# shangfuu/avse_challenge

Measured on AMD Instinct MI355X. Metric: utterances/sec (3s@16kHz + 75 lip frames), higher is better.
Workload: dtype fp32; 1 GPU; avse1 AV baseline train step (BASELINE configs[1]): HIP STFT front-end + AVNet (ResNet18 lip enc + TCN, dilated Conv2d audio net, LSTM fusion) fwd/bwd + Adam; global_batch=32, per_gpu_batch=32, seq_len=48000, stft_frames=376, lip_frames=75, lip_hw=96, parallelism=dp1, hip_graph=fwd+bwd+opt

## Files before the change

### avse_challenge_amd/_lib.py

```python
import ctypes
import os

import torch

_HERE = os.path.dirname(os.path.abspath(__file__))
LIB_PATH = os.environ.get("AVSE_HIP_LIB", os.path.join(_HERE, "libavse_hip.so"))

c_i64, c_i32, c_f32, c_vp = ctypes.c_int64, ctypes.c_int32, ctypes.c_float, ctypes.c_void_p

AVSE_F32, AVSE_BF16 = 0, 1


class ScanFwdArgs(ctypes.Structure):
    _fields_ = [
        ("batch", c_i64), ("dim", c_i64), ("seqlen", c_i64), ("dstate", c_i64),
        ("in_dtype", c_i32), ("delta_softplus", c_i32), ("reverse", c_i32),
        ("u", c_vp), ("u_bs", c_i64), ("u_ds", c_i64),
        ("delta", c_vp), ("delta_bs", c_i64), ("delta_ds", c_i64),
        ("A", c_vp),
        ("B", c_vp), ("B_bs", c_i64), ("B_ns", c_i64),
        ("C", c_vp), ("C_bs", c_i64), ("C_ns", c_i64),
        ("D", c_vp),
        ("z", c_vp), ("z_bs", c_i64), ("z_ds", c_i64),
        ("delta_bias", c_vp),
# ... 167 lines not shown
    "avse_dwconv_gln_fwd": (c_i32, [c_i64] * 5 + [c_vp] * 5 + [c_f32] + [c_vp] * 5),
    "avse_dwconv_gln_fwd_q": (c_i32, [c_i64] * 5 + [c_vp] * 5 + [c_f32] + [c_vp] * 3 + [c_i64] + [c_vp] * 4),
    "avse_dwconv_gln_bwd": (c_i32, [c_i64] * 5 + [c_vp] * 14),
    "avse_prelu_gln_fwd_len": (c_i32, [c_i64] * 3 + [c_vp] * 5 + [c_f32] + [c_vp] * 4),
    "avse_dwconv_gln_fwd_len": (c_i32, [c_i64] * 5 + [c_vp] * 6 + [c_f32] + [c_vp] * 5),
    "avse_dwconv_gln_fwd_q_len": (c_i32, [c_i64] * 5 + [c_vp] * 6 + [c_f32] + [c_vp] * 3 + [c_i64] + [c_vp] * 4),
    "avse_dwconv_fwd_len": (c_i32, [c_i64] * 5 + [c_vp] * 5),
    "avse_upsample_linear_len": (c_i32, [c_i64] * 5 + [c_vp, c_i64, c_i64, c_vp, c_vp, c_vp, c_i64, c_i64, c_vp]),
    "avse_lstm_padded_hidden": (c_i64, [c_i64]),
    "avse_lstm_group_size": (c_i64, [c_i64, c_i64]),
    "avse_lstm_group_workspace_bytes": (c_i64, [c_i64, c_i64]),
    "avse_lstm_group_capacity": (c_i64, [c_i64, c_i32]),
    "avse_lstm_fwd_group": (c_i32, [c_i64, c_i64, c_i64, c_i32, c_vp, c_vp, c_vp, c_i64, c_i64, c_vp, c_vp, c_vp, c_vp,
                                    c_vp]),
    "avse_lstm_bwd_group": (c_i32, [c_i64, c_i64, c_i64, c_i32, c_vp, c_i64, c_i64, c_vp, c_vp, c_vp, c_vp, c_vp, c_vp,
                                    c_vp]),
    "avse_lstm_fwd": (c_i32, [c_i64, c_i64, c_i64, c_i32, c_vp, c_vp, c_vp, c_i64, c_i64, c_vp, c_vp, c_vp]),
    "avse_lstm_bwd": (c_i32, [c_i64, c_i64, c_i64, c_i32, c_vp, c_i64, c_i64, c_vp, c_vp, c_vp, c_vp, c_vp]),
    "avse_gemm_bf16": (c_i32, [ctypes.POINTER(GemmBf16Args), c_vp]),
    "avse_gemm_f32s": (c_i32, [ctypes.POINTER(GemmF32sArgs), c_vp]),
    "avse_split16_planes": (c_i32, [c_i64, c_i64, c_i64, c_vp, c_i64, c_i64, c_vp, c_vp, c_vp, c_vp]),
    "avse_add_max": (c_i32, [c_i64, c_i64, c_i64, c_vp, c_vp, c_vp, c_vp, c_vp]),
    "avse_split16_planes_known": (c_i32, [c_i64, c_i64, c_i64, c_vp, c_i64, c_i64, c_vp, c_vp, c_vp, c_vp]),
    "avse_split16_planes_to": (c_i32, [c_i64, c_i64, c_i64, c_vp, c_i64, c_i64, c_vp, c_vp, c_i64, c_i64, c_vp, c_i32,
                                       c_vp]),
    "avse_dconv_wprep_bytes": (c_i64, []),
    "avse_split16": (c_i32, [c_i64, c_vp, c_vp, c_vp, c_vp]),
    "avse_split16_known": (c_i32, [c_i64, c_vp, c_vp, c_vp, c_vp]),
    "avse_dconv_wprep": (c_i32, [c_vp, c_i32, c_vp, c_vp, c_vp]),
    "avse_dconv_fwd": (c_i32, [c_i64, c_i64, c_i64, c_i64, c_vp, c_vp, c_vp, c_vp, c_vp, c_vp]),
    "avse_dconv_wprep2": (c_i32, [c_vp] * 6),
    "avse_dconv_wgrad16_workspace_bytes": (c_i64, [c_i64, c_i64, c_i64]),
    "avse_dconv_wgrad16": (c_i32, [c_i64, c_i64, c_i64, c_i64, c_vp, c_vp, c_vp, c_vp, c_vp, c_vp, c_vp, c_vp]),
    "avse_conv1_fwd": (c_i32, [c_i64] * 3 + [c_vp] * 5),
    "avse_conv1_dgrad": (c_i32, [c_i64] * 3 + [c_vp] * 4),
    "avse_conv1_wgrad_workspace_bytes": (c_i64, [c_i64] * 3),
    "avse_conv1_wgrad": (c_i32, [c_i64] * 3 + [c_vp] * 6),
    "avse_convf_fwd": (c_i32, [c_i64] + [c_vp] * 5),
    "avse_convf_dgrad": (c_i32, [c_i64] + [c_vp] * 4),
    "avse_convf_wgrad_workspace_bytes": (c_i64, [c_i64]),
    "avse_convf_wgrad": (c_i32, [c_i64] + [c_vp] * 6),
    "avse_sconv_wprep_bytes": (c_i64, [c_i64, c_i64]),
    "avse_sconv_wprep": (c_i32, [c_i64, c_i64, c_vp, c_i32, c_vp, c_vp, c_vp]),
    "avse_sconv_fwd": (c_i32, [c_i64] * 6 + [c_vp] * 6),
    "avse_sconv_wgrad_workspace_bytes": (c_i64, [c_i64] * 6),
    "avse_sconv_wgrad": (c_i32, [c_i64] * 6 + [c_vp] * 7),
    "avse_sconv_dgrad2_supported": (c_i32, [c_i64] * 5),
    "avse_sconv_dgrad2": (c_i32, [c_i64] * 5 + [c_vp] * 6),
    "avse_mbstoi_frames": (c_i64, [c_i64]),
    "avse_mbstoi_workspace_bytes": (c_i64, [c_i64, c_i64]),
    "avse_mbstoi_gate": (c_i32, [c_i64, c_i64] + [c_vp] * 7),
    "avse_mbstoi_bands": (c_i32, [c_i64, c_i64] + [c_vp] * 6),
    "avse_mbstoi_ec": (c_i32, [c_i64, c_i64, c_vp, c_i32, c_i64, c_i64] + [c_vp] * 8),
    "avse_mbstoi_score": (c_i32, [c_i64, c_i64, c_vp, c_i32, c_vp, c_vp, c_vp]),
}

_lib = None


class HipLibraryError(RuntimeError):
    pass


ABI_VERSION = 2


# ... 34 lines not shown
```

### avse_challenge_amd/csrc/dconv.hip

```cpp
#include <algorithm>

#include "bnact_cols.h"
#include "common.h"
#include "split16.h"

namespace avse {
namespace dcf {

typedef _Float16 half8 __attribute__((ext_vector_type(8)));
typedef float floatx16 __attribute__((ext_vector_type(16)));

constexpr int C = 64, KS = 5, NQ = 4, TP = 256, THREADS = 256, WAVES = THREADS / 64;
constexpr int ROWB = 64;
constexpr int WIMG = KS * C * ROWB;
constexpr int NSTG = KS * NQ;
constexpr int MAXD = 16;
constexpr int XIMG_MAX = (TP + 8 * MAXD) * ROWB;
constexpr int STAGE = XIMG_MAX + WIMG;
constexpr int NBUF = 3;
constexpr int MAXP = (XIMG_MAX + WIMG) / 1024 / WAVES + 1;
static_assert(NBUF * STAGE <= 160 * 1024, "LDS");

__device__ inline int swz(int r) { return (r >> 2) & 3; }

// ... 158 lines not shown
    const float scale = __builtin_ldexpf(1.f, -(split_exp(a.maxbits[0]) + split_exp(a.maxbits[1])));
    auto store = [&](int j) {
        const int o = 32 * j + (lane & 31);
        const float bv = a.bias ? a.bias[o] : 0.f;
#pragma unroll
        for (int i = 0; i < 2; ++i)
#pragma unroll
            for (int g = 0; g < 4; ++g)
#pragma unroll
                for (int e = 0; e < 4; ++e) {
                    const int p = p0 + 64 * wave + 32 * i + 8 * g + 4 * (lane >> 5) + e;
                    const float v = acc[i][j][4 * g + e] * scale + bv;
                    if constexpr (EPI != 0) acc[i][j][4 * g + e] = v;
                    if (p < HW) a.y[((int64_t)n * HW + p) * C + o] = v;
                }
    };
    if constexpr (EPI == 0) {
#pragma unroll
        for (int j = 0; j < 2; ++j) store(j);
    } else {
        constexpr int ENQ = EPI == 2 ? 4 : 3;
        float* part = reinterpret_cast<float*>(lds);
        __syncthreads();
        bnact::bn_epi_wave<bnact::ACT_RELU, EPI == 2>(
            a.bn, [&](int i, int j, int r) { return acc[i][j][r]; }, store, (int64_t)n * HW + p0 + 64 * wave,
            (int64_t)(n + 1) * HW, 0, C, lane, part + wave * ENQ * 64);
        __syncthreads();
        bnact::bn_epi_row<EPI == 2>(a.bn, part, NW, 1, (int64_t)bid, 0, C);
    }
}

constexpr int WG_CHUNK = 64;
constexpr int PIXB = 256;
constexpr int WTHREADS = 512, WWAVES = WTHREADS / 64;

typedef short s4_t __attribute__((ext_vector_type(4)));
typedef __attribute__((address_space(3))) s4_t lds_s4_t;

__device__ inline int tswz(int r, int c) { return c ^ (((r & 1) << 1) | ((r & 2) << 2)); }

__device__ inline half8 tfrag(const uint8_t* img, const int (&row)[2], int cb, int pl, int lane) {
    const int g = lane >> 4, i = lane & 15;
    const int q = 2 * cb + (g & 1);
    s4_t v[2];
#pragma unroll
    for (int u = 0; u < 2; ++u) {
        const int r = row[u];
        const int byte = q * 64 + pl * 32 + 8 * (i & 3);
        const int off = r * PIXB + 16 * tswz(r, byte >> 4) + (byte & 15);
        v[u] = __builtin_amdgcn_ds_read_tr16_b64_v4i16((lds_s4_t*)(img + off));
    }
    const s4_t w0 = v[0], w1 = v[1];
    const short __attribute__((ext_vector_type(8))) w = {w0[0], w0[1], w0[2], w0[3], w1[0], w1[1], w1[2], w1[3]};
    return __builtin_bit_cast(half8, w);
}

struct WArgs {
    const void* xq;
    const void* dyq;
    const uint32_t* xmax;
    const uint32_t* dymax;
    float* part;
    float* dbpart;
    int N, H, W, cpi, chunks, ranges;
};

struct ChunkPos {
    int n, p0, hA, wA0;
    __device__ void init(int c, int cpi, int W) {
        n = c / cpi;
        p0 = (c - n * cpi) * WG_CHUNK;
        hA = p0 / W;
        wA0 = p0 - hA * W;
    }
    __device__ void next(int HW, int W) {
        p0 += WG_CHUNK;
        if (p0 >= HW) {
            ++n;
            p0 = hA = wA0 = 0;
        } else {
            wA0 += WG_CHUNK;
            if (wA0 >= W) {
                wA0 -= W;
                ++hA;
            }
        }
    }
};

template <int D>
__global__ __launch_bounds__(WTHREADS, 1) void wgrad_kernel(WArgs a) {
    constexpr int NP = WG_CHUNK + 8 * D;
    constexpr int YIMG = WG_CHUNK * PIXB, XIMG = NP * PIXB, STG = YIMG + XIMG;
    constexpr int NB = (3 * STG <= 160 * 1024) ? 3 : 2;
    constexpr int PY = YIMG / 1024, PT = PY + XIMG / 1024;
    constexpr int MAXPW = PT / WWAVES + 1;
    __shared__ __attribute__((aligned(1024))) uint8_t lds[NB * STG];
    const int lane = threadIdx.x & 63;
    const int wave = __builtin_amdgcn_readfirstlane(threadIdx.x >> 6);
    const int bid = xcd_remap(blockIdx.x, gridDim.x);
    const int r = bid / KS, kh = bid % KS;
    const int c_lo = (int)((int64_t)r * a.chunks / a.ranges), c_hi = (int)((int64_t)(r + 1) * a.chunks / a.ranges);
    const int HW = a.H * a.W;
    const i4_t rx = dma_rsrc(a.xq, (int64_t)a.N * HW * PIXB);
    const i4_t ry = dma_rsrc(a.dyq, (int64_t)a.N * HW * PIXB);
    const uint32_t lds0 = lds_u32(lds);
    const int npieces = (PT - wave + WWAVES - 1) / WWAVES;
    const int pr = lane >> 4, pc = lane & 15;
    int pj[MAXPW];
    uint32_t psw[MAXPW];
#pragma unroll
    for (int m = 0; m < MAXPW; ++m) {
        const int k = wave + WWAVES * m;
        pj[m] = k < PY ? 4 * k + pr : 4 * (k - PY) + pr;
        psw[m] = 16u * tswz(pj[m], pc);
    }

    auto issue = [&](const ChunkPos& cp, int buf) {
        const int nA = min(WG_CHUNK, a.W - cp.wA0);
        const int row1 = cp.hA + D * (kh - 2), row2 = nA < WG_CHUNK ? row1 + 1 : -1000000;
        const int ybase = cp.n * HW + cp.p0;
        const int nHrow = cp.n * a.H;
        const uint32_t img = lds0 + buf * STG;
#pragma unroll
        for (int m = 0; m < MAXPW; ++m) {
            if (m >= npieces) break;
            const int k = wave + WWAVES * m;
            if (k < PY) {
                const int j = pj[m];
                const uint32_t off = cp.p0 + j < HW ? (uint32_t)(ybase + j) * PIXB + psw[m] : 0x7FFFFFF0u;
                dma16(ry, img + k * 1024, off);
            } else {
                const int q = pj[m];
                const bool s1 = q < nA + 4 * D;
                const int col = s1 ? cp.wA0 - 2 * D + q : q - nA - 6 * D;
                const int row = s1 ? row1 : row2;
                const bool ok = (unsigned)col < (unsigned)a.W && (unsigned)row < (unsigned)a.H;
                const uint32_t pix = (uint32_t)((nHrow + row) * a.W + col);
                dma16(rx, img + YIMG + (k - PY) * 1024, ok ? pix * PIXB + psw[m] : 0x7FFFFFF0u);
            }
        }
    };

    const int half = wave >> 2, ob = (wave >> 1) & 1, ib = wave & 1;
    const bool want_db = a.dbpart != nullptr && kh == 0 && ib == 0;
    floatx16 acc[KS], accb;
#pragma unroll
    for (int k = 0; k < KS; ++k)
#pragma unroll
        for (int e = 0; e < 16; ++e) acc[k][e] = 0.f;
#pragma unroll
    for (int e = 0; e < 16; ++e) accb[e] = 0.f;
    half8 ones;
#pragma unroll
    for (int e = 0; e < 8; ++e) ones[e] = (_Float16)1.0f;

    const int g = lane >> 4, li = lane & 15;
    ChunkPos cc, ci;
    cc.init(c_lo, a.cpi, a.W);
    ci = cc;
    if (c_lo < c_hi) {
        issue(ci, 0);
        ci.next(HW, a.W);
    }
    if (NB == 3 && c_lo + 1 < c_hi) {
        issue(ci, 1);
        ci.next(HW, a.W);
    }
    for (int c = c_lo; c < c_hi; ++c) {
        const int it = c - c_lo;
        const bool ahead = NB == 3 && c + 1 < c_hi;
        if (ahead) wait_all_but(npieces);
        else asm volatile("s_waitcnt vmcnt(0)" ::: "memory");
        __builtin_amdgcn_s_barrier();
        asm volatile("" ::: "memory");
        if (c + NB - 1 < c_hi) {
            issue(ci, (it + NB - 1) % NB);
            ci.next(HW, a.W);
        }
        const uint8_t* yimg = lds + (it % NB) * STG;
        const uint8_t* ximg = yimg + YIMG;
        const int nA = min(WG_CHUNK, a.W - cc.wA0);
#pragma unroll
        for (int s2 = 0; s2 < 2; ++s2) {
            const int s = 2 * half + s2;
            int ry_[2], rx_[2];
#pragma unroll
            for (int u = 0; u < 2; ++u) {
                const int j = 16 * s + 8 * (g >> 1) + (li >> 2) + 4 * u;
                ry_[u] = j;
                rx_[u] = j < nA ? j : j + 4 * D;
            }
            const half8 ah = tfrag(yimg, ry_, ob, 0, lane), al = tfrag(yimg, ry_, ob, 1, lane);
#pragma unroll
            for (int kw = 0; kw < KS; ++kw) {
                const int rk[2] = {rx_[0] + D * kw, rx_[1] + D * kw};
                const half8 bh = tfrag(ximg, rk, ib, 0, lane), bl = tfrag(ximg, rk, ib, 1, lane);
                acc[kw] = __builtin_amdgcn_mfma_f32_32x32x16_f16(ah, bh, acc[kw], 0, 0, 0);
                acc[kw] = __builtin_amdgcn_mfma_f32_32x32x16_f16(ah, bl, acc[kw], 0, 0, 0);
                acc[kw] = __builtin_amdgcn_mfma_f32_32x32x16_f16(al, bh, acc[kw], 0, 0, 0);
            }
            if (want_db) {
                accb = __builtin_amdgcn_mfma_f32_32x32x16_f16(ah, ones, accb, 0, 0, 0);
                accb = __builtin_amdgcn_mfma_f32_32x32x16_f16(al, ones, accb, 0, 0, 0);
            }
        }
        cc.next(HW, a.W);
    }
    const float sc = __builtin_ldexpf(1.f, -(split_exp(*a.xmax) + split_exp(*a.dymax)));
    float* pp = a.part + (((int64_t)r * 2 + half) * KS + kh) * KS * C * C;
#pragma unroll
    for (int kw = 0; kw < KS; ++kw)
#pragma unroll
        for (int q = 0; q < 4; ++q)
#pragma unroll
            for (int e = 0; e < 4; ++e) {
                const int o = 32 * ob + 8 * q + 4 * (lane >> 5) + e, i = 32 * ib + (lane & 31);
                pp[((int64_t)kw * C + o) * C + i] = acc[kw][4 * q + e] * sc;
            }
    if (want_db && (lane & 31) == 0) {
        const float sd = __builtin_ldexpf(1.f, -split_exp(*a.dymax));
#pragma unroll
        for (int q = 0; q < 4; ++q)
#pragma unroll
            for (int e = 0; e < 4; ++e)
                a.dbpart[((int64_t)r * 2 + half) * C + 32 * ob + 8 * q + 4 * (lane >> 5) + e] = accb[4 * q + e] * sd;
    }
}

__global__ void wgrad_reduce_kernel(const float* __restrict__ part, const float* __restrict__ dbpart, int slabs,
                                    float* __restrict__ dw, float* __restrict__ db) {
    constexpr int TOTAL = KS * KS * C * C;
    const int idx = blockIdx.x * blockDim.x + threadIdx.x;
    if (idx >= TOTAL) {
        if (db != nullptr && idx < TOTAL + C) {
            float v = 0.f;
            for (int g = 0; g < slabs; ++g) v += dbpart[(int64_t)g * C + idx - TOTAL];
            db[idx - TOTAL] = v;
        }
        return;
    }
    float v = 0.f;
    for (int g = 0; g < slabs; ++g) v += part[(int64_t)g * TOTAL + idx];
    const int i = idx % C, o = (idx / C) % C, kw = (idx / (C * C)) % KS, kh = idx / (KS * C * C);
    dw[((o * C + i) * KS + kh) * KS + kw] = v;
}

inline int wgrad_ranges(int chunks) { return std::max(1, std::min(chunks, 256 / KS * 1)); }

constexpr int AMAX_NT = 1024, AMAX_GRID = 256;
__global__ __launch_bounds__(AMAX_NT) void absmax_kernel(const float4* x, int64_t n4, uint32_t* out) {
    __shared__ uint32_t red[AMAX_NT / 64];
    float m = 0.f;
    const int64_t stride = (int64_t)gridDim.x * AMAX_NT;
    for (int64_t i0 = blockIdx.x * (int64_t)AMAX_NT + threadIdx.x; i0 < n4; i0 += 4 * stride) {
        float4 v[4];
#pragma unroll
        for (int u = 0; u < 4; ++u) v[u] = i0 + u * stride < n4 ? x[i0 + u * stride] : make_float4(0.f, 0.f, 0.f, 0.f);
#pragma unroll
        for (int u = 0; u < 4; ++u) m = fmaxf(m, fmaxf(fmaxf(fabsf(v[u].x), fabsf(v[u].y)), fmaxf(fabsf(v[u].z), fabsf(v[u].w))));
    }
    block_max_publish<AMAX_NT / 64>(m, red, out);
}

__global__ void split_kernel(const float* x, int64_t nq, const uint32_t* maxbits, uint4* xq) {
    const float sc = split_scale(maxbits[0]);
    for (int64_t i = blockIdx.x * (int64_t)blockDim.x + threadIdx.x; i < nq; i += (int64_t)gridDim.x * blockDim.x) {
        const float4* s = reinterpret_cast<const float4*>(x + i * 16);
        uint32_t hi[8], lo[8];
#pragma unroll
        for (int k = 0; k < 4; ++k) {
            const float4 v = s[k];
            hi[2 * k] = split_pair(v.x, v.y, sc, lo[2 * k]);
            hi[2 * k + 1] = split_pair(v.z, v.w, sc, lo[2 * k + 1]);
        }
        uint4* d = xq + i * 4;
        d[0] = uint4{hi[0], hi[1], hi[2], hi[3]};
        d[1] = uint4{hi[4], hi[5], hi[6], hi[7]};
        d[2] = uint4{lo[0], lo[1], lo[2], lo[3]};
        d[3] = uint4{lo[4], lo[5], lo[6], lo[7]};
    }
// ... 67 lines not shown
    AVSE_CHECK_LAUNCH();
    return AVSE_OK;
}

int avse_split16_known(int64_t n_pix, const float* x, void* xq, const uint32_t* maxbits, avse_stream_t stream) {
    if (!x || !xq || !maxbits) return AVSE_EINVAL;
    if (n_pix <= 0) return AVSE_ESHAPE;
    if (((uintptr_t)x & 15) || ((uintptr_t)xq & 15)) return AVSE_EALIGN;
    const int64_t nq = n_pix * NQ;
    const int blocks = (int)std::min<int64_t>((nq + 255) / 256, 8192);
    hipLaunchKernelGGL(split_kernel, dim3(blocks), dim3(256), 0, (hipStream_t)stream, x, nq, maxbits,
                       reinterpret_cast<uint4*>(xq));
    AVSE_CHECK_LAUNCH();
    return AVSE_OK;
}

int avse_dconv_wprep(const float* w, int32_t transposed, void* wq, uint32_t* maxbits, avse_stream_t stream) {
    if (!w || !wq || !maxbits) return AVSE_EINVAL;
    hipLaunchKernelGGL(wprep_kernel, dim3(1), dim3(1024), 0, (hipStream_t)stream, w, transposed, maxbits,
                       reinterpret_cast<uint16_t*>(wq));
    AVSE_CHECK_LAUNCH();
    return AVSE_OK;
}

int avse_dconv_wprep2(const float* w, void* wq, void* wq_t, uint32_t* maxbits, uint32_t* maxbits_t,
                      avse_stream_t stream) {
    if (!w || !wq || !maxbits || (wq_t == nullptr) != (maxbits_t == nullptr)) return AVSE_EINVAL;
    hipLaunchKernelGGL(wprep2_kernel, dim3(wq_t ? 2 * NSTG : NSTG), dim3(1024), 0, (hipStream_t)stream, w, maxbits,
                       maxbits_t, reinterpret_cast<uint16_t*>(wq), reinterpret_cast<uint16_t*>(wq_t));
    AVSE_CHECK_LAUNCH();
    return AVSE_OK;
}

int64_t avse_dconv_wgrad16_workspace_bytes(int64_t N, int64_t H, int64_t W) {
    const int64_t chunks = N * ((H * W + WG_CHUNK - 1) / WG_CHUNK);
    return 4 * 2 * (int64_t)wgrad_ranges((int)std::min<int64_t>(chunks, 1 << 30)) * (KS * KS * C * C + C);
}

int avse_dconv_wgrad16(int64_t N, int64_t H, int64_t W, int64_t dil, const void* xq, const uint32_t* xmax,
                       const void* dyq, const uint32_t* dymax, float* dw, float* db, float* workspace,
                       avse_stream_t stream) {
    if (!xq || !xmax || !dyq || !dymax || !dw || !workspace) return AVSE_EINVAL;
    if (N <= 0 || H <= 0 || W < WG_CHUNK || (dil != 2 && dil != 4 && dil != 8 && dil != 16)) return AVSE_ESHAPE;
    if (N * H * W * 256 >= (1LL << 31) - 1024) return AVSE_ESHAPE;
    WArgs a;
    a.xq = xq;
    a.dyq = dyq;
    a.xmax = xmax;
    a.dymax = dymax;
    a.N = (int)N;
    a.H = (int)H;
    a.W = (int)W;
    a.cpi = (int)((H * W + WG_CHUNK - 1) / WG_CHUNK);
    a.chunks = (int)(N * a.cpi);
    a.ranges = wgrad_ranges(a.chunks);
    a.part = workspace;
    a.dbpart = db ? workspace + (int64_t)2 * a.ranges * KS * KS * C * C : nullptr;
    const dim3 grid((unsigned)(a.ranges * KS)), block(WTHREADS);
    hipStream_t st = (hipStream_t)stream;
    switch (dil) {
        case 2: hipLaunchKernelGGL(wgrad_kernel<2>, grid, block, 0, st, a); break;
        case 4: hipLaunchKernelGGL(wgrad_kernel<4>, grid, block, 0, st, a); break;
        case 8: hipLaunchKernelGGL(wgrad_kernel<8>, grid, block, 0, st, a); break;
        default: hipLaunchKernelGGL(wgrad_kernel<16>, grid, block, 0, st, a); break;
    }
    AVSE_CHECK_LAUNCH();
    constexpr int TOTAL = KS * KS * C * C;
    hipLaunchKernelGGL(wgrad_reduce_kernel, dim3((TOTAL + C + 255) / 256), dim3(256), 0, st, a.part, a.dbpart,
                       2 * a.ranges, dw, db);
    AVSE_CHECK_LAUNCH();
    return AVSE_OK;
}

static inline int dcf_nw(int64_t dil) { return dil <= 8 ? 4 : 8; }

int64_t avse_dconv_bn_rows(int64_t N, int64_t H, int64_t W, int64_t dil) {
    if (N <= 0 || H <= 0 || W < 256) return 0;
    return N * ((H * W + 64 * dcf_nw(dil) - 1) / (64 * dcf_nw(dil)));
}

static int dconv_launch(int64_t N, int64_t H, int64_t W, int64_t dil, const void* xq, const void* wq,
                        const uint32_t* maxbits, const float* bias, float* y, const avse::bnact::BnEpi* bn, int epi,
                        avse_stream_t stream);

int avse_dconv_fwd(int64_t N, int64_t H, int64_t W, int64_t dil, const void* xq, const void* wq,
                   const uint32_t* maxbits, const float* bias, float* y, avse_stream_t stream) {
    return dconv_launch(N, H, W, dil, xq, wq, maxbits, bias, y, nullptr, 0, stream);
}

int avse_dconv_dgrad_bn(int64_t N, int64_t H, int64_t W, int64_t dil, const void* dyq, const void* wq_t,
                        const uint32_t* maxbits, float* dx, const float* bn_x, const float* bn_stats,
                        const float* gamma, const float* beta, int32_t act, int32_t want_max, float* rows,
                        avse_stream_t stream) {
    if (!bn_x || !bn_stats || !rows) return AVSE_EINVAL;
    if (act != avse::bnact::ACT_RELU) return AVSE_ESHAPE;
    avse::bnact::BnEpi bn;
    bn.x = bn_x;
    bn.stats = bn_stats;
    bn.gamma = gamma;
    bn.beta = beta;
    bn.alpha = nullptr;
    bn.alpha_n = 0;
// ... 42 lines not shown
```

### include/avse_hip.h

```cpp
#ifndef AVSE_HIP_H
#define AVSE_HIP_H

#include <stdint.h>

#ifdef __cplusplus
extern "C" {
#endif

typedef void* avse_stream_t;

enum { AVSE_OK = 0, AVSE_EINVAL = -1, AVSE_ESHAPE = -2, AVSE_EDTYPE = -3, AVSE_ELAUNCH = -4, AVSE_EALIGN = -5,
       AVSE_ENORESIDENT = -6 };
enum { AVSE_F32 = 0, AVSE_BF16 = 1, AVSE_U8 = 2 };

const char* avse_strerror(int code);
int avse_abi_version(void);

typedef struct {
    int64_t batch, dim, seqlen, dstate;
    int32_t in_dtype;
    int32_t delta_softplus;
    int32_t reverse;
    const void* u;      int64_t u_bs, u_ds;
    const void* delta;  int64_t delta_bs, delta_ds;
// ... 321 lines not shown
int avse_convf_dgrad(int64_t npix, const float* dy, const float* w, float* dx, avse_stream_t stream);
int64_t avse_convf_wgrad_workspace_bytes(int64_t npix);
int avse_convf_wgrad(int64_t npix, const float* x, const float* dy, float* dw, float* db, float* workspace,
                     avse_stream_t stream);

int64_t avse_sconv_wprep_bytes(int64_t co, int64_t ci);
int avse_sconv_wprep(int64_t co, int64_t ci, const float* w, int32_t transposed, void* wq, uint32_t* wmax,
                     avse_stream_t stream);
int avse_sconv_fwd(int64_t N, int64_t Hi, int64_t Wi, int64_t ci, int64_t co, int64_t stride, const void* xq,
                   const uint32_t* xmax, const void* wq, const uint32_t* wmax, float* y, avse_stream_t stream);
int64_t avse_sconv_wgrad_workspace_bytes(int64_t N, int64_t Hi, int64_t Wi, int64_t ci, int64_t co, int64_t stride);
int avse_sconv_dgrad2_supported(int64_t N, int64_t Hi, int64_t Wi, int64_t ci, int64_t co);
int avse_sconv_dgrad2(int64_t N, int64_t Hi, int64_t Wi, int64_t ci, int64_t co, const void* dyq,
                      const uint32_t* dymax, const void* wq, const uint32_t* wmax, float* dx, avse_stream_t stream);
int avse_sconv_wgrad(int64_t N, int64_t Hi, int64_t Wi, int64_t ci, int64_t co, int64_t stride, const void* xq,
                     const uint32_t* xmax, const void* dyq, const uint32_t* dymax, float* dw, float* workspace,
                     avse_stream_t stream);
int avse_dconv_fwd(int64_t N, int64_t H, int64_t W, int64_t dil, const void* xq, const void* wq,
                   const uint32_t* maxbits, const float* bias, float* y, avse_stream_t stream);
int64_t avse_dconv_bn_rows(int64_t N, int64_t H, int64_t W, int64_t dil);
int avse_dconv_dgrad_bn(int64_t N, int64_t H, int64_t W, int64_t dil, const void* dyq, const void* wq_t,
                        const uint32_t* maxbits, float* dx, const float* bn_x, const float* bn_stats,
                        const float* gamma, const float* beta, int32_t act, int32_t want_max, float* rows,
                        avse_stream_t stream);
int64_t avse_sconv_bn_rows(int64_t N, int64_t H, int64_t W, int64_t co);
int avse_sconv_dgrad1_bn(int64_t N, int64_t H, int64_t W, int64_t ci, int64_t co, const void* dyq,
                         const uint32_t* dymax, const void* wq_t, const uint32_t* wmax, float* dx, const float* bn_x,
                         const float* bn_stats, const float* gamma, const float* beta, int32_t act, const float* alpha,
                         int32_t alpha_n, int32_t want_max, float* rows, avse_stream_t stream);
int64_t avse_dconv_wgrad16_workspace_bytes(int64_t N, int64_t H, int64_t W);
int avse_dconv_wgrad16(int64_t N, int64_t H, int64_t W, int64_t dil, const void* xq, const uint32_t* xmax,
                       const void* dyq, const uint32_t* dymax, float* dw, float* db, float* workspace,
                       avse_stream_t stream);

int64_t avse_mbstoi_frames(int64_t len);
int64_t avse_mbstoi_workspace_bytes(int64_t batch, int64_t max_len);
int avse_mbstoi_gate(int64_t batch, int64_t max_len, const double* sig, const int32_t* len, const double* window,
                     double* workspace, int32_t* kept, int32_t* count, avse_stream_t stream);
int avse_mbstoi_bands(int64_t batch, int64_t max_len, const double* sig, const double* window, const int32_t* kept,
                      const int32_t* count, double* bq, avse_stream_t stream);
int avse_mbstoi_ec(int64_t batch, int64_t frame_slots, const int32_t* frames, int32_t frames_offset, int64_t n_taus,
                   int64_t n_gammas, const double* bq, const double* tau_table, const double* gamma_table, double* d,
                   double* d_ec_or_null, double* p_ec_or_null, int32_t* winner_or_null, avse_stream_t stream);
int avse_mbstoi_score(int64_t batch, int64_t frame_slots, const int32_t* frames, int32_t frames_offset, const double* d,
                      double* score, avse_stream_t stream);

#ifdef __cplusplus
}
#endif
#endif
```

Measured before the change: 480.0 utt/s.

## Rewrite dilated conv wgrad as row-streaming kernel with sliding x-row ring

Replaces the chunked dilated-conv weight-gradient kernel, where each block handled one kh and re-read input rows, with a row-streaming kernel. Each work unit covers (n, column chunk, row phase), and a 6-slot LDS ring holds the input rows so all 25 taps are computed from each loaded dy row. DMA of the next rows is interleaved with the MFMAs, and fragment loads are software-pipelined. The taps are split across waves 13/12. The aim is less redundant global/LDS traffic and better overlap, at the cost of more complex scheduling, a different reduction-slab count, and a new plan query entry point.

```diff
diff --git a/avse_challenge_amd/_lib.py b/avse_challenge_amd/_lib.py
--- a/avse_challenge_amd/_lib.py
+++ b/avse_challenge_amd/_lib.py
@@ -223,6 +223,7 @@
     "avse_dconv_wprep2": (c_i32, [c_vp] * 6),
     "avse_dconv_wgrad16_workspace_bytes": (c_i64, [c_i64, c_i64, c_i64]),
     "avse_dconv_wgrad16": (c_i32, [c_i64, c_i64, c_i64, c_i64, c_vp, c_vp, c_vp, c_vp, c_vp, c_vp, c_vp, c_vp]),
+    "avse_dconv_wgrad16_plan": (c_i32, [c_i64, c_i64, c_i64, c_i64, c_vp]),
     "avse_conv1_fwd": (c_i32, [c_i64] * 3 + [c_vp] * 5),
     "avse_conv1_dgrad": (c_i32, [c_i64] * 3 + [c_vp] * 4),
     "avse_conv1_wgrad_workspace_bytes": (c_i64, [c_i64] * 3),
diff --git a/avse_challenge_amd/csrc/dconv.hip b/avse_challenge_amd/csrc/dconv.hip
--- a/avse_challenge_amd/csrc/dconv.hip
+++ b/avse_challenge_amd/csrc/dconv.hip
@@ -214,201 +214,11 @@
 
 constexpr int WG_CHUNK = 64;
 constexpr int PIXB = 256;
-constexpr int WTHREADS = 512, WWAVES = WTHREADS / 64;
 
 typedef short s4_t __attribute__((ext_vector_type(4)));
 typedef __attribute__((address_space(3))) s4_t lds_s4_t;
 
 __device__ inline int tswz(int r, int c) { return c ^ (((r & 1) << 1) | ((r & 2) << 2)); }
-
-__device__ inline half8 tfrag(const uint8_t* img, const int (&row)[2], int cb, int pl, int lane) {
-    const int g = lane >> 4, i = lane & 15;
-    const int q = 2 * cb + (g & 1);
-    s4_t v[2];
-#pragma unroll
-    for (int u = 0; u < 2; ++u) {
-        const int r = row[u];
-        const int byte = q * 64 + pl * 32 + 8 * (i & 3);
-        const int off = r * PIXB + 16 * tswz(r, byte >> 4) + (byte & 15);
-        v[u] = __builtin_amdgcn_ds_read_tr16_b64_v4i16((lds_s4_t*)(img + off));
-    }
-    const s4_t w0 = v[0], w1 = v[1];
-    const short __attribute__((ext_vector_type(8))) w = {w0[0], w0[1], w0[2], w0[3], w1[0], w1[1], w1[2], w1[3]};
-    return __builtin_bit_cast(half8, w);
-}
-
-struct WArgs {
-    const void* xq;
-    const void* dyq;
-    const uint32_t* xmax;
-    const uint32_t* dymax;
-    float* part;
-    float* dbpart;
-    int N, H, W, cpi, chunks, ranges;
-};
-
-struct ChunkPos {
-    int n, p0, hA, wA0;
-    __device__ void init(int c, int cpi, int W) {
-        n = c / cpi;
-        p0 = (c - n * cpi) * WG_CHUNK;
-        hA = p0 / W;
-        wA0 = p0 - hA * W;
-    }
-    __device__ void next(int HW, int W) {
-        p0 += WG_CHUNK;
-        if (p0 >= HW) {
-            ++n;
-            p0 = hA = wA0 = 0;
-        } else {
-            wA0 += WG_CHUNK;
-            if (wA0 >= W) {
-                wA0 -= W;
-                ++hA;
-            }
-        }
-    }
-};
-
-template <int D>
-__global__ __launch_bounds__(WTHREADS, 1) void wgrad_kernel(WArgs a) {
-    constexpr int NP = WG_CHUNK + 8 * D;
-    constexpr int YIMG = WG_CHUNK * PIXB, XIMG = NP * PIXB, STG = YIMG + XIMG;
-    constexpr int NB = (3 * STG <= 160 * 1024) ? 3 : 2;
-    constexpr int PY = YIMG / 1024, PT = PY + XIMG / 1024;
-    constexpr int MAXPW = PT / WWAVES + 1;
-    __shared__ __attribute__((aligned(1024))) uint8_t lds[NB * STG];
-    const int lane = threadIdx.x & 63;
-    const int wave = __builtin_amdgcn_readfirstlane(threadIdx.x >> 6);
-    const int bid = xcd_remap(blockIdx.x, gridDim.x);
-    const int r = bid / KS, kh = bid % KS;
-    const int c_lo = (int)((int64_t)r * a.chunks / a.ranges), c_hi = (int)((int64_t)(r + 1) * a.chunks / a.ranges);
-    const int HW = a.H * a.W;
-    const i4_t rx = dma_rsrc(a.xq, (int64_t)a.N * HW * PIXB);
-    const i4_t ry = dma_rsrc(a.dyq, (int64_t)a.N * HW * PIXB);
-    const uint32_t lds0 = lds_u32(lds);
-    const int npieces = (PT - wave + WWAVES - 1) / WWAVES;
-    const int pr = lane >> 4, pc = lane & 15;
-    int pj[MAXPW];
-    uint32_t psw[MAXPW];
-#pragma unroll
-    for (int m = 0; m < MAXPW; ++m) {
-        const int k = wave + WWAVES * m;
-        pj[m] = k < PY ? 4 * k + pr : 4 * (k - PY) + pr;
-        psw[m] = 16u * tswz(pj[m], pc);
-    }
-
-    auto issue = [&](const ChunkPos& cp, int buf) {
-        const int nA = min(WG_CHUNK, a.W - cp.wA0);
-        const int row1 = cp.hA + D * (kh - 2), row2 = nA < WG_CHUNK ? row1 + 1 : -1000000;
-        const int ybase = cp.n * HW + cp.p0;
-        const int nHrow = cp.n * a.H;
-        const uint32_t img = lds0 + buf * STG;
-#pragma unroll
-        for (int m = 0; m < MAXPW; ++m) {
-            if (m >= npieces) break;
-            const int k = wave + WWAVES * m;
-            if (k < PY) {
-                const int j = pj[m];
-                const uint32_t off = cp.p0 + j < HW ? (uint32_t)(ybase + j) * PIXB + psw[m] : 0x7FFFFFF0u;
-                dma16(ry, img + k * 1024, off);
-            } else {
-                const int q = pj[m];
-                const bool s1 = q < nA + 4 * D;
-                const int col = s1 ? cp.wA0 - 2 * D + q : q - nA - 6 * D;
-                const int row = s1 ? row1 : row2;
-                const bool ok = (unsigned)col < (unsigned)a.W && (unsigned)row < (unsigned)a.H;
-                const uint32_t pix = (uint32_t)((nHrow + row) * a.W + col);
-                dma16(rx, img + YIMG + (k - PY) * 1024, ok ? pix * PIXB + psw[m] : 0x7FFFFFF0u);
-            }
-        }
-    };
-
-    const int half = wave >> 2, ob = (wave >> 1) & 1, ib = wave & 1;
-    const bool want_db = a.dbpart != nullptr && kh == 0 && ib == 0;
-    floatx16 acc[KS], accb;
-#pragma unroll
-    for (int k = 0; k < KS; ++k)
-#pragma unroll
-        for (int e = 0; e < 16; ++e) acc[k][e] = 0.f;
-#pragma unroll
-    for (int e = 0; e < 16; ++e) accb[e] = 0.f;
-    half8 ones;
-#pragma unroll
-    for (int e = 0; e < 8; ++e) ones[e] = (_Float16)1.0f;
-
-    const int g = lane >> 4, li = lane & 15;
-    ChunkPos cc, ci;
-    cc.init(c_lo, a.cpi, a.W);
-    ci = cc;
-    if (c_lo < c_hi) {
-        issue(ci, 0);
-        ci.next(HW, a.W);
-    }
-    if (NB == 3 && c_lo + 1 < c_hi) {
-        issue(ci, 1);
-        ci.next(HW, a.W);
-    }
-    for (int c = c_lo; c < c_hi; ++c) {
-        const int it = c - c_lo;
-        const bool ahead = NB == 3 && c + 1 < c_hi;
-        if (ahead) wait_all_but(npieces);
-        else asm volatile("s_waitcnt vmcnt(0)" ::: "memory");
-        __builtin_amdgcn_s_barrier();
-        asm volatile("" ::: "memory");
-        if (c + NB - 1 < c_hi) {
-            issue(ci, (it + NB - 1) % NB);
-            ci.next(HW, a.W);
-        }
-        const uint8_t* yimg = lds + (it % NB) * STG;
-        const uint8_t* ximg = yimg + YIMG;
-        const int nA = min(WG_CHUNK, a.W - cc.wA0);
-#pragma unroll
-        for (int s2 = 0; s2 < 2; ++s2) {
-            const int s = 2 * half + s2;
-            int ry_[2], rx_[2];
-#pragma unroll
-            for (int u = 0; u < 2; ++u) {
-                const int j = 16 * s + 8 * (g >> 1) + (li >> 2) + 4 * u;
-                ry_[u] = j;
-                rx_[u] = j < nA ? j : j + 4 * D;
-            }
-            const half8 ah = tfrag(yimg, ry_, ob, 0, lane), al = tfrag(yimg, ry_, ob, 1, lane);
-#pragma unroll
-            for (int kw = 0; kw < KS; ++kw) {
-                const int rk[2] = {rx_[0] + D * kw, rx_[1] + D * kw};
-                const half8 bh = tfrag(ximg, rk, ib, 0, lane), bl = tfrag(ximg, rk, ib, 1, lane);
-                acc[kw] = __builtin_amdgcn_mfma_f32_32x32x16_f16(ah, bh, acc[kw], 0, 0, 0);
-                acc[kw] = __builtin_amdgcn_mfma_f32_32x32x16_f16(ah, bl, acc[kw], 0, 0, 0);
-                acc[kw] = __builtin_amdgcn_mfma_f32_32x32x16_f16(al, bh, acc[kw], 0, 0, 0);
-            }
-            if (want_db) {
-                accb = __builtin_amdgcn_mfma_f32_32x32x16_f16(ah, ones, accb, 0, 0, 0);
-                accb = __builtin_amdgcn_mfma_f32_32x32x16_f16(al, ones, accb, 0, 0, 0);
-            }
-        }
-        cc.next(HW, a.W);
-    }
-    const float sc = __builtin_ldexpf(1.f, -(split_exp(*a.xmax) + split_exp(*a.dymax)));
-    float* pp = a.part + (((int64_t)r * 2 + half) * KS + kh) * KS * C * C;
-#pragma unroll
-    for (int kw = 0; kw < KS; ++kw)
-#pragma unroll
-        for (int q = 0; q < 4; ++q)
-#pragma unroll
-            for (int e = 0; e < 4; ++e) {
-                const int o = 32 * ob + 8 * q + 4 * (lane >> 5) + e, i = 32 * ib + (lane & 31);
-                pp[((int64_t)kw * C + o) * C + i] = acc[kw][4 * q + e] * sc;
-            }
-    if (want_db && (lane & 31) == 0) {
-        const float sd = __builtin_ldexpf(1.f, -split_exp(*a.dymax));
-#pragma unroll
-        for (int q = 0; q < 4; ++q)
-#pragma unroll
-            for (int e = 0; e < 4; ++e)
-                a.dbpart[((int64_t)r * 2 + half) * C + 32 * ob + 8 * q + 4 * (lane >> 5) + e] = accb[4 * q + e] * sd;
-    }
-}
 
 __global__ void wgrad_reduce_kernel(const float* __restrict__ part, const float* __restrict__ dbpart, int slabs,
                                     float* __restrict__ dw, float* __restrict__ db) {
@@ -428,7 +238,271 @@
     dw[((o * C + i) * KS + kh) * KS + kw] = v;
 }
 
-inline int wgrad_ranges(int chunks) { return std::max(1, std::min(chunks, 256 / KS * 1)); }
+
+namespace rows {
+
+constexpr int RTHREADS = 256;
+constexpr int XPIXB = 128;
+constexpr int CWMAX = 80;
+constexpr int NSLOT = 6;
+constexpr int YBUF = CWMAX * PIXB;
+constexpr int TAPS0 = 13;
+constexpr int MAXWG = 256;
+
+constexpr int slot_bytes(int D) { return (CWMAX + 4 * D) * XPIXB; }
+constexpr int lds_bytes(int D) { return NSLOT * slot_bytes(D) + 2 * YBUF; }
+static_assert(lds_bytes(MAXD) <= 160 * 1024, "LDS");
+static_assert(slot_bytes(2) % 1024 == 0, "whole DMA pieces");
+
+inline __host__ __device__ int chunks_of(int W) { return W / 64 + (W % 64 > 16 ? 1 : 0); }
+
+struct Plan {
+    int nck, nwg, slabs, lds;
+    int64_t units, steps, pieces;
+};
+
+inline Plan make_plan(int64_t N, int64_t H, int64_t W, int D) {
+    Plan p;
+    p.nck = chunks_of((int)W);
+    p.units = N * p.nck * D * 2;
+    p.nwg = (int)std::min<int64_t>(MAXWG, p.units);
+    p.slabs = p.nwg / 2;
+    p.lds = lds_bytes(D);
+    p.steps = 0;
+    p.pieces = 0;
+    for (int c = 0; c < p.nck; ++c) {
+        const int cw = c == p.nck - 1 ? (int)W - 64 * c : 64, ks = (cw + 15) / 16, npx = (16 * ks + 4 * D) / 8;
+        for (int rho = 0; rho < D; ++rho) {
+            const int64_t T = rho < H ? (H - rho + D - 1) / D : 0;
+            if (T == 0) continue;
+            p.steps += 2 * N * T;
+            p.pieces += 2 * N * ((T + 4) * npx + T * 4 * ks);
+        }
+    }
+    return p;
+}
+
+struct RArgs {
+    const void* xq;
+    const void* dyq;
+    const uint32_t* xmax;
+    const uint32_t* dymax;
+    float* part;
+    float* dbpart;
+    int N, H, W, nck, units;
+};
+
+struct LaneOff {
+    uint32_t x[2][2], y[2][2];
+    __device__ void init(int lane, int ob) {
+        const int g = lane >> 4, i = lane & 15;
+#pragma unroll
+        for (int u = 0; u < 2; ++u)
+#pragma unroll
+            for (int pl = 0; pl < 2; ++pl) {
+                const int p = 8 * (g >> 1) + (i >> 2) + 4 * u;
+                const int bx = (g & 1) * 64 + pl * 32 + 8 * (i & 3);
+                x[u][pl] = (uint32_t)(p * XPIXB + 16 * ((bx >> 4) ^ (p & 2)) + (bx & 15));
+                const int by = (2 * ob + (g & 1)) * 64 + pl * 32 + 8 * (i & 3);
+                y[u][pl] = (uint32_t)(p * PIXB + 16 * tswz(p, by >> 4) + (by & 15));
+            }
+    }
+};
+
+template <int OFF>
+__device__ __forceinline__ half8 frag2(uint32_t a0, uint32_t a1) {
+    const s4_t w0 = __builtin_amdgcn_ds_read_tr16_b64_v4i16((lds_s4_t*)(uintptr_t)(a0 + OFF));
+    const s4_t w1 = __builtin_amdgcn_ds_read_tr16_b64_v4i16((lds_s4_t*)(uintptr_t)(a1 + OFF));
+    const short __attribute__((ext_vector_type(8))) w = {w0[0], w0[1], w0[2], w0[3], w1[0], w1[1], w1[2], w1[3]};
+    return __builtin_bit_cast(half8, w);
+}
+
+struct Frags {
+    half8 ah, al, bh, bl;
+};
+
+__device__ __forceinline__ void load_a(const LaneOff& lo, uint32_t ybase, half8& ah, half8& al) {
+    ah = frag2<0>(ybase + lo.y[0][0], ybase + lo.y[1][0]);
+    al = frag2<0>(ybase + lo.y[0][1], ybase + lo.y[1][1]);
+}
+
+template <int D, int TAP>
+__device__ __forceinline__ void load_b(const LaneOff& lo, const uint32_t (&xbase)[KS], half8& bh, half8& bl) {
+    constexpr int KH = TAP / KS, KW = TAP % KS, F_ = ((D * KW) >> 1) & 1, O_ = D * KW * XPIXB;
+    const uint32_t xb = xbase[KH];
+    bh = frag2<O_>(xb + lo.x[0][F_], xb + lo.x[1][F_]);
+    bl = frag2<O_>(xb + lo.x[0][1 - F_], xb + lo.x[1][1 - F_]);
+}
+
+template <int D, int T0, int T1, bool ISSUE, typename F>
+__device__ __forceinline__ void kstep(floatx16 (&acc)[TAPS0], floatx16& accb, const LaneOff& lo, uint32_t ybase,
+                                      const uint32_t (&xbase)[KS], bool want_db, F&& piece, Frags& f, bool has_next) {
+    const half8 ah = f.ah, al = f.al;
+    half8 bh = f.bh, bl = f.bl;
+#pragma unroll
+    for (int tap = T0; tap < T1; ++tap) {
+        half8 nh = bh, nl = bl;
+        if (tap + 1 < T1) {
+#define AVSE_ROWS_NEXT(K) case T0 + K: load_b<D, (T0 + K + 1 < KS * KS ? T0 + K + 1 : 0)>(lo, xbase, nh, nl); break;
+            switch (tap) {
+                AVSE_ROWS_NEXT(0) AVSE_ROWS_NEXT(1) AVSE_ROWS_NEXT(2) AVSE_ROWS_NEXT(3) AVSE_ROWS_NEXT(4)
+                AVSE_ROWS_NEXT(5) AVSE_ROWS_NEXT(6) AVSE_ROWS_NEXT(7) AVSE_ROWS_NEXT(8) AVSE_ROWS_NEXT(9)
+                AVSE_ROWS_NEXT(10) AVSE_ROWS_NEXT(11)
+                default: break;
+            }
+#undef AVSE_ROWS_NEXT
+        } else if (has_next) {
+            uint32_t xn[KS];
+#pragma unroll
+            for (int kh = 0; kh < KS; ++kh) xn[kh] = xbase[kh] + 16 * XPIXB;
+            load_a(lo, ybase + 16 * PIXB, f.ah, f.al);
+            load_b<D, T0>(lo, xn, f.bh, f.bl);
+        }
+        __builtin_amdgcn_sched_barrier(0);
+        acc[tap - T0] = __builtin_amdgcn_mfma_f32_32x32x16_f16(ah, bh, acc[tap - T0], 0, 0, 0);
+        acc[tap - T0] = __builtin_amdgcn_mfma_f32_32x32x16_f16(ah, bl, acc[tap - T0], 0, 0, 0);
+        acc[tap - T0] = __builtin_amdgcn_mfma_f32_32x32x16_f16(al, bh, acc[tap - T0], 0, 0, 0);
+        if constexpr (ISSUE) {
+            if (tap - T0 < 10) piece(tap - T0);
+        }
+        bh = nh;
+        bl = nl;
+    }
+    if (want_db) {
+        half8 ones;
+#pragma unroll
+        for (int e = 0; e < 8; ++e) ones[e] = (_Float16)1.0f;
+        accb = __builtin_amdgcn_mfma_f32_32x32x16_f16(ah, ones, accb, 0, 0, 0);
+        accb = __builtin_amdgcn_mfma_f32_32x32x16_f16(al, ones, accb, 0, 0, 0);
+    }
+}
+
+template <int D, int TS>
+__device__ __forceinline__ void wave_body(const RArgs& a, uint8_t* lds, int wave, int lane) {
+    constexpr int SLOTB = slot_bytes(D), RING = NSLOT * SLOTB;
+    constexpr int T0 = TS == 0 ? 0 : TAPS0, T1 = TS == 0 ? TAPS0 : KS * KS, ts = TS;
+    const int nwg = gridDim.x;
+    const int bid = xcd_remap(blockIdx.x, nwg);
+    const int ib = bid & 1, ob = wave & 1;
+    const int HW = a.H * a.W;
+    const i4_t rx = dma_rsrc(a.xq, (int64_t)a.N * HW * PIXB);
+    const i4_t ry = dma_rsrc(a.dyq, (int64_t)a.N * HW * PIXB);
+    const uint32_t lds0 = lds_u32(lds);
+    const int ypx0 = 4 * wave + (lane >> 4), xpos0 = 8 * wave + (lane >> 3);
+    const uint32_t ysw = 16u * tswz(lane >> 4, lane & 15);
+    const uint32_t xsw = (uint32_t)(ib * XPIXB) + 16u * ((lane & 7) ^ ((lane >> 3) & 2));
+    const bool want_db = TS == 1 && a.dbpart != nullptr && ib == 0;
+    LaneOff lo;
+    lo.init(lane, ob);
+
+    floatx16 acc[TAPS0], accb;
+#pragma unroll
+    for (int k = 0; k < TAPS0; ++k)
+#pragma unroll
+        for (int e = 0; e < 16; ++e) acc[k][e] = 0.f;
+#pragma unroll
+    for (int e = 0; e < 16; ++e) accb[e] = 0.f;
+
+    for (int u = bid; u < a.units; u += nwg) {
+        int rest = u >> 1;
+        const int cc = rest % a.nck;
+        rest /= a.nck;
+        const int rho = rest % D, n = rest / D;
+        const int T = rho < a.H ? (a.H - rho + D - 1) / D : 0;
+        if (T == 0) continue;
+        const int w0 = 64 * cc, cw = cc == a.nck - 1 ? a.W - w0 : 64;
+        const int ks = (cw + 15) >> 4, npx = (16 * ks + 4 * D) >> 3;
+        const int nH = n * a.H;
+        auto dma_y = [&](int m, int t) {
+            const int px = ypx0 + 16 * m;
+            const int pix = (nH + rho + t * D) * a.W + w0 + px;
+            dma16(ry, lds0 + RING + (t & 1) * YBUF + (wave + 4 * m) * 1024,
+                  px < cw ? (uint32_t)pix * PIXB + ysw : 0x7FFFFFF0u);
+        };
+        auto dma_x = [&](int m, int tau, int slot) {
+            const int row = rho + tau * D, col = w0 - 2 * D + xpos0 + 32 * m;
+            const bool ok = tau >= 0 && row < a.H && (unsigned)col < (unsigned)a.W;
+            const int pix = (nH + row) * a.W + col;
+            dma16(rx, lds0 + slot * SLOTB + (wave + 4 * m) * 1024, ok ? (uint32_t)pix * PIXB + xsw : 0x7FFFFFF0u);
+        };
+        __builtin_amdgcn_s_barrier();
+        asm volatile("" ::: "memory");
+#pragma unroll 1
+        for (int tau = -2; tau <= 2; ++tau)
+            for (int m = 0; wave + 4 * m < npx; ++m) dma_x(m, tau, tau + 2);
+        for (int m = 0; m < ks; ++m) dma_y(m, 0);
+        int s0 = 0;
+#pragma unroll 1
+        for (int t = 0; t < T; ++t) {
+            asm volatile("s_waitcnt vmcnt(0)" ::: "memory");
+            __builtin_amdgcn_s_barrier();
+            asm volatile("" ::: "memory");
+            int sb[KS];
+#pragma unroll
+            for (int kh = 0; kh < KS; ++kh) sb[kh] = (s0 + kh >= NSLOT ? s0 + kh - NSLOT : s0 + kh) * SLOTB;
+            const int snew = s0 + 5 >= NSLOT ? s0 + 5 - NSLOT : s0 + 5;
+            const bool more = t + 1 < T;
+            auto piece = [&](int k) {
+                if (!more) return;
+                const int m = k >> 1;
+                if (k & 1) {
+                    if (wave + 4 * m < npx) dma_x(m, t + 3, snew);
+                } else {
+                    if (m < ks) dma_y(m, t + 1);
+                }
+            };
+            const uint32_t ybuf = lds0 + RING + (t & 1) * YBUF;
+            uint32_t xb[KS];
+#pragma unroll
+            for (int kh = 0; kh < KS; ++kh) xb[kh] = lds0 + sb[kh];
+            Frags f;
+            load_a(lo, ybuf, f.ah, f.al);
+            load_b<D, T0>(lo, xb, f.bh, f.bl);
+            kstep<D, T0, T1, true>(acc, accb, lo, ybuf, xb, want_db, piece, f, ks > 1);
+#pragma unroll 1
+            for (int s = 1; s < ks; ++s) {
+#pragma unroll
+                for (int kh = 0; kh < KS; ++kh) xb[kh] += 16 * XPIXB;
+                kstep<D, T0, T1, false>(acc, accb, lo, ybuf + s * 16 * PIXB, xb, want_db, piece, f, s + 1 < ks);
+            }
+            s0 = s0 + 1 >= NSLOT ? 0 : s0 + 1;
+        }
+    }
+
+    const float sc = __builtin_ldexpf(1.f, -(split_exp(*a.xmax) + split_exp(*a.dymax)));
+    float* pp = a.part + ((int64_t)(bid >> 1) * KS * KS + TAPS0 * ts) * C * C;
+#pragma unroll
+    for (int k = 0; k < TAPS0; ++k) {
+        if (k < T1 - T0) {
+#pragma unroll
+            for (int q = 0; q < 4; ++q)
+#pragma unroll
+                for (int e = 0; e < 4; ++e) {
+                    const int o = 32 * ob + 8 * q + 4 * (lane >> 5) + e, i = 32 * ib + (lane & 31);
+                    pp[((int64_t)k * C + o) * C + i] = acc[k][4 * q + e] * sc;
+                }
+        }
+    }
+    if (want_db && (lane & 31) == 0) {
+        const float sd = __builtin_ldexpf(1.f, -split_exp(*a.dymax));
+#pragma unroll
+        for (int q = 0; q < 4; ++q)
+#pragma unroll
+            for (int e = 0; e < 4; ++e)
+                a.dbpart[(int64_t)(bid >> 1) * C + 32 * ob + 8 * q + 4 * (lane >> 5) + e] = accb[4 * q + e] * sd;
+    }
+}
+
+template <int D>
+__global__ __launch_bounds__(RTHREADS, 1) void wgrad_rows_kernel(RArgs a) {
+    __shared__ __attribute__((aligned(1024))) uint8_t lds[lds_bytes(D)];
+    const int lane = threadIdx.x & 63;
+    const int wave = __builtin_amdgcn_readfirstlane(threadIdx.x >> 6);
+    if (wave < 2) wave_body<D, 0>(a, lds, wave, lane);
+    else wave_body<D, 1>(a, lds, wave, lane);
+}
+
+}
 
 constexpr int AMAX_NT = 1024, AMAX_GRID = 256;
 __global__ __launch_bounds__(AMAX_NT) void absmax_kernel(const float4* x, int64_t n4, uint32_t* out) {
@@ -562,18 +636,36 @@
     return AVSE_OK;
 }
 
+static bool wgrad16_shape_ok(int64_t N, int64_t H, int64_t W, int64_t dil) {
+    if (N <= 0 || H <= 0 || W < WG_CHUNK || (dil != 2 && dil != 4 && dil != 8 && dil != 16)) return false;
+    return N * H * W * 256 < (1LL << 31) - 1024;
+}
+
 int64_t avse_dconv_wgrad16_workspace_bytes(int64_t N, int64_t H, int64_t W) {
-    const int64_t chunks = N * ((H * W + WG_CHUNK - 1) / WG_CHUNK);
-    return 4 * 2 * (int64_t)wgrad_ranges((int)std::min<int64_t>(chunks, 1 << 30)) * (KS * KS * C * C + C);
+    if (!wgrad16_shape_ok(N, H, W, MAXD)) return 0;
+    return 4 * (int64_t)rows::make_plan(N, H, W, MAXD).slabs * (KS * KS * C * C + C);
+}
+
+int avse_dconv_wgrad16_plan(int64_t N, int64_t H, int64_t W, int64_t dil, int64_t out[6]) {
+    if (!out) return AVSE_EINVAL;
+    if (!wgrad16_shape_ok(N, H, W, dil)) return AVSE_ESHAPE;
+    const rows::Plan p = rows::make_plan(N, H, W, (int)dil);
+    out[0] = p.units;
+    out[1] = p.steps;
+    out[2] = p.pieces;
+    out[3] = p.slabs;
+    out[4] = p.lds;
+    out[5] = p.nwg;
+    return AVSE_OK;
 }
 
 int avse_dconv_wgrad16(int64_t N, int64_t H, int64_t W, int64_t dil, const void* xq, const uint32_t* xmax,
                        const void* dyq, const uint32_t* dymax, float* dw, float* db, float* workspace,
                        avse_stream_t stream) {
     if (!xq || !xmax || !dyq || !dymax || !dw || !workspace) return AVSE_EINVAL;
-    if (N <= 0 || H <= 0 || W < WG_CHUNK || (dil != 2 && dil != 4 && dil != 8 && dil != 16)) return AVSE_ESHAPE;
-    if (N * H * W * 256 >= (1LL << 31) - 1024) return AVSE_ESHAPE;
-    WArgs a;
+    if (!wgrad16_shape_ok(N, H, W, dil)) return AVSE_ESHAPE;
+    const rows::Plan p = rows::make_plan(N, H, W, (int)dil);
+    rows::RArgs a;
     a.xq = xq;
     a.dyq = dyq;
     a.xmax = xmax;
@@ -581,23 +673,22 @@
     a.N = (int)N;
     a.H = (int)H;
     a.W = (int)W;
-    a.cpi = (int)((H * W + WG_CHUNK - 1) / WG_CHUNK);
-    a.chunks = (int)(N * a.cpi);
-    a.ranges = wgrad_ranges(a.chunks);
+    a.nck = p.nck;
+    a.units = (int)p.units;
     a.part = workspace;
-    a.dbpart = db ? workspace + (int64_t)2 * a.ranges * KS * KS * C * C : nullptr;
-    const dim3 grid((unsigned)(a.ranges * KS)), block(WTHREADS);
+    a.dbpart = db ? workspace + (int64_t)p.slabs * KS * KS * C * C : nullptr;
+    const dim3 grid((unsigned)p.nwg), block(rows::RTHREADS);
     hipStream_t st = (hipStream_t)stream;
     switch (dil) {
-        case 2: hipLaunchKernelGGL(wgrad_kernel<2>, grid, block, 0, st, a); break;
-        case 4: hipLaunchKernelGGL(wgrad_kernel<4>, grid, block, 0, st, a); break;
-        case 8: hipLaunchKernelGGL(wgrad_kernel<8>, grid, block, 0, st, a); break;
-        default: hipLaunchKernelGGL(wgrad_kernel<16>, grid, block, 0, st, a); break;
+        case 2: hipLaunchKernelGGL(rows::wgrad_rows_kernel<2>, grid, block, 0, st, a); break;
+        case 4: hipLaunchKernelGGL(rows::wgrad_rows_kernel<4>, grid, block, 0, st, a); break;
+        case 8: hipLaunchKernelGGL(rows::wgrad_rows_kernel<8>, grid, block, 0, st, a); break;
+        default: hipLaunchKernelGGL(rows::wgrad_rows_kernel<16>, grid, block, 0, st, a); break;
     }
     AVSE_CHECK_LAUNCH();
     constexpr int TOTAL = KS * KS * C * C;
-    hipLaunchKernelGGL(wgrad_reduce_kernel, dim3((TOTAL + C + 255) / 256), dim3(256), 0, st, a.part, a.dbpart,
-                       2 * a.ranges, dw, db);
+    hipLaunchKernelGGL(wgrad_reduce_kernel, dim3((TOTAL + C + 255) / 256), dim3(256), 0, st, a.part, a.dbpart, p.slabs,
+                       dw, db);
     AVSE_CHECK_LAUNCH();
     return AVSE_OK;
 }
diff --git a/include/avse_hip.h b/include/avse_hip.h
--- a/include/avse_hip.h
+++ b/include/avse_hip.h
@@ -377,6 +377,7 @@
 int avse_dconv_wgrad16(int64_t N, int64_t H, int64_t W, int64_t dil, const void* xq, const uint32_t* xmax,
                        const void* dyq, const uint32_t* dymax, float* dw, float* db, float* workspace,
                        avse_stream_t stream);
+int avse_dconv_wgrad16_plan(int64_t N, int64_t H, int64_t W, int64_t dil, int64_t out[6]);
 
 int64_t avse_mbstoi_frames(int64_t len);
 int64_t avse_mbstoi_workspace_bytes(int64_t batch, int64_t max_len);
```

Result: faster. 493.3 utt/s (median of 6 runs) (+2.8%).
